# mynameisfiber/baton

Hardware: NVIDIA H100
Metric: federated local samples/sec (whole box), ResNet-18 FedAvg, synthetic non-IID 32x32 shards (higher is better)
Workload: dtype bf16

## Files before the change

### baton_b200/build_ext.py

```python
from __future__ import annotations

import os
import shutil
import subprocess
import sys
import sysconfig
import time
from concurrent.futures import ThreadPoolExecutor

HERE = os.path.dirname(os.path.abspath(__file__))
CSRC = os.path.join(HERE, "csrc")
BUILD = os.path.join(HERE, "csrc", "build")
TRACE = os.environ.get("BATON_BUILD_TRACE") == "1"
if TRACE:
    BUILD = os.path.join(HERE, "csrc", "build_trace")
TARGET = os.path.join(HERE, "_C_trace.so" if TRACE else "_C.so")

CU_SOURCES = ["gemm_wgmma.cu", "gemm_fp8.cu", "quant.cu", "attention.cu", "im2col_tma.cu", "gemm_simt.cu", "fedavg.cu", "elementwise.cu", "conv.cu", "norm.cu", "loss.cu"]
HEADERS = ["ptx.cuh", "launch.h", "pdl.cuh", "mx.cuh", "sgd.cuh", "dp.cuh"]
NVCC_FLAGS = ["-gencode", "arch=compute_90a,code=sm_90a", "-lineinfo", "-O3", "-std=c++17",
              "-Xcompiler", "-fPIC", "--use_fast_math", "-Xptxas", "-v"]
if os.environ.get("BATON_BUILD_PHASE_TIMING") == "1":
    NVCC_FLAGS.append("-DB200_FEDAVG_PHASE_TIMING")
if TRACE:
    NVCC_FLAGS += ["-DB200_TRACE", "-DB200_FEDAVG_PHASE_TIMING"]


def _nvcc() -> str:
    for cand in (os.environ.get("CUDA_HOME", "") + "/bin/nvcc", "/usr/local/cuda/bin/nvcc", shutil.which("nvcc") or ""):
        if cand and os.path.exists(cand):
            return cand
    raise RuntimeError("nvcc not found")


# ... 72 lines not shown
```

### baton_b200/csrc/bindings.cpp

```cpp
#include <ATen/cuda/CUDAContext.h>
#include <c10/cuda/CUDAGuard.h>
#include <torch/extension.h>

#include <optional>
#include <vector>

#include "launch.h"

namespace {

inline cudaStream_t cur_stream() { return at::cuda::getCurrentCUDAStream().stream(); }
inline void check(int rc, const char* what) {
  TORCH_CHECK(rc == 0, "baton_b200::", what, " failed with code ", rc,
              rc > 0 ? std::string(" (") + cudaGetErrorString(static_cast<cudaError_t>(rc)) + ")" : std::string());
}
inline const void* cptr(const at::Tensor& t) { return t.data_ptr(); }
inline void* ptr(at::Tensor& t) { return t.data_ptr(); }
template <class T>
inline T* opt_ptr(const std::optional<at::Tensor>& t) {
  return (t.has_value() && t->defined()) ? reinterpret_cast<T*>(t->data_ptr()) : nullptr;
}
#define CHECK_CUDA(x) TORCH_CHECK((x).is_cuda(), #x " must be a CUDA tensor")

inline const float* prox_anchor(const std::optional<at::Tensor>& anchor, int64_t numel, const at::Tensor& hyper) {
// ... 31 lines not shown
              "affine epilogue: fp32 [N] scale / shift");
  long long ldr = 0;
  if (residual.has_value() && residual->defined()) {
    CHECK_CUDA(*residual);
    TORCH_CHECK(residual->scalar_type() == at::kBFloat16 && residual->stride(-1) == 1 && residual->size(-1) == N &&
                    residual->numel() >= rows * N,
                "affine epilogue: bf16 [rows, N] residual with unit inner stride");
    ldr = residual->dim() >= 2 ? residual->stride(-2) : N;
  }
  return B200AffineEpilogue{scale->data_ptr<float>(), shift->data_ptr<float>(), opt_ptr<const void>(residual), ldr,
                            relu ? 1 : 0};
}

extern "C" {
#define B200_TRACE_TUS(X) X(gemm_wgmma) X(gemm_fp8) X(quant) X(attention) X(im2col_tma) X(gemm_simt) X(fedavg) \
  X(elementwise) X(conv) X(norm) X(loss)
#define B200_DECL(tu) int b200_trace_set_##tu(unsigned long long* p);
B200_TRACE_TUS(B200_DECL)
#undef B200_DECL
}
bool trace_set(const std::optional<at::Tensor>& buf) {
  unsigned long long* p = nullptr;
  if (buf.has_value() && buf->defined()) {
    CHECK_CUDA(*buf);
    TORCH_CHECK(buf->scalar_type() == at::kLong && buf->is_contiguous() && buf->numel() >= 4, "trace buffer: int64 [2+2n]");
    p = reinterpret_cast<unsigned long long*>(buf->data_ptr());
  }
  int rc = 0;
#define B200_SET(tu) rc |= b200_trace_set_##tu(p);
  B200_TRACE_TUS(B200_SET)
#undef B200_SET
// ... 116 lines not shown
  return true;
}
bool conv_igemm_dgrad(const at::Tensor& dy, const at::Tensor& w, at::Tensor dx, int64_t kh, int64_t kw, int64_t pad,
                      int64_t cluster_k, int64_t force_bn) {
  CHECK_CUDA(dy); CHECK_CUDA(w); CHECK_CUDA(dx);
  TORCH_CHECK(dy.scalar_type() == at::kBFloat16 && w.scalar_type() == at::kBFloat16 && dx.scalar_type() == at::kBFloat16 &&
              dy.dim() == 4 && dx.dim() == 4 && dy.is_contiguous() && w.is_contiguous() && dx.is_contiguous());
  const c10::cuda::CUDAGuard guard(dy.device());
  const int rc = b200_conv_igemm_dgrad(cptr(dy), cptr(w), ptr(dx), static_cast<int>(dx.size(0)), static_cast<int>(dx.size(1)),
                                       static_cast<int>(dx.size(2)), static_cast<int>(dx.size(3)), static_cast<int>(dy.size(3)),
                                       static_cast<int>(kh), static_cast<int>(kw), static_cast<int>(pad),
                                       static_cast<int>(dy.size(1)), static_cast<int>(dy.size(2)),
                                       static_cast<int>(cluster_k), static_cast<int>(force_bn), cur_stream());
  if (rc == -2) return false;
  check(rc, "conv_igemm_dgrad");
  return true;
}
bool conv_igemm_dgrad_s2(const at::Tensor& dy, const at::Tensor& w, at::Tensor dx, int64_t kh, int64_t kw,
                         const std::vector<int64_t>& ntaps, const std::vector<int64_t>& taps, int64_t force_bn) {
  CHECK_CUDA(dy); CHECK_CUDA(w); CHECK_CUDA(dx);
  TORCH_CHECK(dy.scalar_type() == at::kBFloat16 && w.scalar_type() == at::kBFloat16 && dx.scalar_type() == at::kBFloat16 &&
              dy.dim() == 4 && dx.dim() == 4 && dy.is_contiguous() && w.is_contiguous() && dx.is_contiguous());
  TORCH_CHECK(ntaps.size() == 4 && taps.size() == 16, "conv_igemm_dgrad_s2: 4 classes x 4 taps");
  int nt[4], tw[16];
  for (int i = 0; i < 4; ++i) nt[i] = static_cast<int>(ntaps[i]);
  for (int i = 0; i < 16; ++i) tw[i] = static_cast<int>(taps[i]);
  const c10::cuda::CUDAGuard guard(dy.device());
  const int rc = b200_conv_igemm_dgrad_s2(cptr(dy), cptr(w), ptr(dx), static_cast<int>(dx.size(0)),
                                          static_cast<int>(dx.size(1)), static_cast<int>(dx.size(2)),
                                          static_cast<int>(dx.size(3)), static_cast<int>(dy.size(3)), static_cast<int>(kh),
// ... 534 lines not shown
}

PYBIND11_MODULE(TORCH_EXTENSION_NAME, m) {
  m.doc() = "baton_b200 sm_90a kernels";
  m.attr("MAX_RANKS") = B200_MAX_RANKS;
  m.def("gemm", &gemm);
  m.def("trace_set", &trace_set);
  m.def("attention_fwd", &attention_fwd);
  m.def("attention_bwd", &attention_bwd);
  m.def("bn_bwd_cluster", &bn_bwd_cluster);
  m.def("im2col_tma_probe", &im2col_tma_probe);
  m.def("conv_igemm_fwd", &conv_igemm_fwd);
  m.def("conv_igemm_wgrad", &conv_igemm_wgrad);
  m.def("conv_igemm_dgrad", &conv_igemm_dgrad);
  m.def("conv_igemm_dgrad_s2", &conv_igemm_dgrad_s2);
  m.def("gemm_batched", &gemm_batched);
  m.def("gemm_fp8", &gemm_fp8);
  m.def("quant_mx_rows", &quant_mx_rows);
  m.def("quant_mx_cols", &quant_mx_cols);
  m.def("dequant_mx", &dequant_mx);
  m.def("fused_sgd", &fused_sgd);
  m.def("fused_sgd_segments", &fused_sgd_segments);
  m.def("weighted_sum", &weighted_sum);
  m.def("fold_client", &fold_client);
  m.def("cast", &cast);
  m.def("gather_rows", &gather_rows);
  m.def("colsum", &colsum);
  m.def("add_bf16", &add_bf16);
  m.def("relu_bwd", &relu_bwd);
  m.def("gelu", &gelu);
// ... 31 lines not shown
```

### baton_b200/csrc/gemm_wgmma.cu

```cuda
#define B200_TU_TAG 1
#include "ptx.cuh"
#include "launch.h"
#include "pdl.cuh"
#include "sgd.cuh"

namespace b200 {

constexpr int BM = 128;
constexpr int BK = 64;
constexpr int WG_K = 16;
constexpr int GEMM_THREADS = 384;
constexpr int CONSUMER_WARPS = 8;
constexpr int CONSUMER_THREADS = 32 * CONSUMER_WARPS;
constexpr int MAX_STAGES = 8;
constexpr int S2_MAX_TAPS = 4;

struct GemmParams {
  int M, N, K;
  void* D;
  long long ldd;
  const float* bias;
  int out_fp32;
  int act;
  float* col_stats;
// ... 51 lines not shown
  static constexpr int STAGE_BYTES = A_BYTES + B_BYTES;
  static constexpr int PART_PITCH = BN + 4;
  static constexpr int PART_BYTES = BM * PART_PITCH * 4;
};

__device__ __forceinline__ float apply_act(float v, int act) {
  if (act == 1) return fmaxf(v, 0.f);
  if (act == 2) {
    const float k0 = 0.7978845608028654f, k1 = 0.044715f;
    float t = tanhf(k0 * (v + k1 * v * v * v));
    return 0.5f * v * (1.f + t);
  }
  return v;
}

__device__ __forceinline__ uint32_t cluster_ctarank() {
  uint32_t r;
  asm volatile("mov.u32 %0, %%cluster_ctarank;" : "=r"(r));
  return r;
}
__device__ __forceinline__ void cluster_sync_all() {
  asm volatile("barrier.cluster.arrive.release.aligned;" ::: "memory");
  asm volatile("barrier.cluster.wait.acquire.aligned;" ::: "memory");
}
__device__ __forceinline__ float4 ld_dsmem_f4(uint32_t local_smem_addr, uint32_t cta_rank) {
  uint32_t remote;
  asm volatile("mapa.shared::cluster.u32 %0, %1, %2;" : "=r"(remote) : "r"(local_smem_addr), "r"(cta_rank));
  float4 v;
  asm volatile("ld.shared::cluster.v4.f32 {%0, %1, %2, %3}, [%4];"
               : "=f"(v.x), "=f"(v.y), "=f"(v.z), "=f"(v.w)
               : "r"(remote)
               : "memory");
  return v;
}

#define COLSUM_STEP(OFF, HALF)                                                  \
  {                                                                             \
    const bool upper = (lane & (OFF)) != 0;                                     \
    _Pragma("unroll") for (int i = 0; i < (HALF); ++i) {                        \
      const float keep = upper ? t[i + (HALF)] : t[i];                          \
      const float send = upper ? t[i] : t[i + (HALF)];                          \
      t[i] = keep + __shfl_xor_sync(0xffffffffu, send, (OFF));                  \
    }                                                                           \
  }
__device__ __forceinline__ float warp_colsum32(float (&t)[32]) {
  const uint32_t lane = lane_id();
  COLSUM_STEP(16, 16) COLSUM_STEP(8, 8) COLSUM_STEP(4, 4) COLSUM_STEP(2, 2) COLSUM_STEP(1, 1)
  return t[0];
}
#undef COLSUM_STEP
__device__ __forceinline__ void accumulate_col_stats(const GemmParams& p, int col0, const float (&v)[32]) {
  float s[32], q[32];
#pragma unroll
  for (int j = 0; j < 32; ++j) {
    const float r = __bfloat162float(__float2bfloat16_rn(v[j]));
    s[j] = r;
    q[j] = r * r;
  }
  const float cs = warp_colsum32(s), cq = warp_colsum32(q);
  const int col = col0 + static_cast<int>(lane_id());
  if (col < p.N) {
    atomicAdd(p.col_stats + col, cs);
    atomicAdd(p.col_stats + p.N + col, cq);
  }
}

__device__ __forceinline__ void stage_col_stats(float* sbuf, int BNv, int c, const float (&v)[32]) {
  float s[32], q[32];
#pragma unroll
  for (int j = 0; j < 32; ++j) {
    const float r = __bfloat162float(__float2bfloat16_rn(v[j]));
    s[j] = r;
    q[j] = r * r;
  }
  const float cs = warp_colsum32(s), cq = warp_colsum32(q);
  const int lane = static_cast<int>(lane_id());
  sbuf[c + lane] = cs;
  sbuf[BNv + c + lane] = cq;
}

template <int NV, int ACT, bool BIAS>
__device__ __forceinline__ void transform_chunk_t(const GemmParams& p, int col0, float (&v)[NV]) {
  float b[NV];
  if (BIAS) {
    if (col0 + NV <= p.N && ((reinterpret_cast<uintptr_t>(p.bias + col0) & 15) == 0)) {
#pragma unroll
      for (int j = 0; j < NV; j += 4) {
        const float4 t = __ldg(reinterpret_cast<const float4*>(p.bias + col0 + j));
        b[j] = t.x; b[j + 1] = t.y; b[j + 2] = t.z; b[j + 3] = t.w;
      }
    } else {
#pragma unroll
      for (int j = 0; j < NV; ++j) b[j] = (col0 + j) < p.N ? __ldg(p.bias + col0 + j) : 0.f;
// ... 964 lines not shown
  if (le != cudaSuccess) return static_cast<int>(le);
  return static_cast<int>(cudaGetLastError());
}

}

extern "C" int b200_encode_map2_bf16(void* map, const void* base, long long rows, long long cols, long long ld,
                                     int box_cols, int box_rows) {
  return b200::make_map(reinterpret_cast<CUtensorMap*>(map), base, rows, cols, ld, box_cols, box_rows);
}
extern "C" int b200_encode_map4_bf16(void* map, const void* base, long long rows, long long cols, long long ld,
                                     long long inner, long long s_inner, long long outer, long long s_outer,
                                     int box_cols, int box_rows) {
  return b200::make_map4(reinterpret_cast<CUtensorMap*>(map), base, rows, cols, ld, inner, s_inner, outer, s_outer,
                         box_cols, box_rows);
}

extern "C" int b200_gemm_bf16(const void* a, const void* b, void* d, const float* bias, int M, int N, int K,
                              long long lda, long long ldb, long long ldd, int a_mn, int b_mn, int out_fp32, int act,
                              int split_k, int accumulate, float alpha, const uint32_t* tile_flags,
                              uint32_t flag_epoch, long long flag_elem_off, int flag_tile_elems,
                              long long flag_bias_off, int force_bn, float* col_stats, const uint32_t* flag_epoch_ptr,
                              const B200SgdEpilogue* sgd, const B200AffineEpilogue* affine, cudaStream_t stream) {
  using namespace b200;
  if (M <= 0 || N <= 0 || K <= 0) return 0;
  if (sgd != nullptr && (!accumulate || !out_fp32 || !a_mn || !b_mn || bias != nullptr || act != 0 || alpha != 1.0f ||
                         col_stats != nullptr || tile_flags != nullptr))
    return B200_SGD_EPILOGUE_DECLINED;
  if (affine != nullptr && (sgd != nullptr || accumulate || out_fp32 || bias != nullptr || act != 0 || alpha != 1.0f ||
                            col_stats != nullptr || tile_flags != nullptr || split_k > 1 || !affine_ok(*affine, N)))
// ... 311 lines not shown
```

### baton_b200/csrc/launch.h

```cpp
#pragma once
#include <cuda_runtime.h>
#include <stdint.h>

#define B200_MAX_RANKS 16

extern "C" {

struct B200SgdEpilogue {
  float* theta;
  void* theta_bf16;
  float* mom;
  const float* hyper;
  int nesterov;
  const float* anchor;
};
#define B200_SGD_EPILOGUE_DECLINED (-6)

struct B200AffineEpilogue {
  const float* scale;
  const float* shift;
  const void* residual;
  long long ldr;
  int relu;
};
// ... 10 lines not shown
                           long long d_outer, long long d_inner, int accumulate, cudaStream_t stream);
int b200_attention_fwd(const void* qkv, void* out, void* probs, int B, int S, int H, int dh, float scale,
                       cudaStream_t stream);
int b200_attention_bwd(const void* qkv, const void* dout, const void* probs, void* dqkv, int B, int S, int H, int dh,
                       float scale, cudaStream_t stream);
int b200_conv_igemm_fwd(const void* x, const void* w, void* y, int N, int H, int W, int Cin, int Cout, int KH, int KW,
                        int stride, int pad, int Ho, int Wo, int cluster_k, int force_bn, float* col_stats,
                        const B200AffineEpilogue* affine, cudaStream_t stream);
int b200_conv_igemm_dgrad(const void* dy, const void* w, void* dx, int N, int H, int W, int Cin, int Cout, int KH, int KW,
                          int pad, int Ho, int Wo, int cluster_k, int force_bn, cudaStream_t stream);
int b200_conv_igemm_dgrad_s2(const void* dy, const void* w, void* dx, int N, int H, int W, int Cin, int Cout, int KH,
                             int KW, int Ho, int Wo, const int* ntaps, const int* taps, int force_bn, cudaStream_t stream);
int b200_conv_igemm_wgrad(const void* dy, const void* x, float* dw, int N, int H, int W, int Cin, int Cout, int KH, int KW,
                          int stride, int pad, int Ho, int Wo, int split_k, int force_bn, const B200SgdEpilogue* sgd,
                          cudaStream_t stream);
int b200_im2col_tma_probe(const void* x, void* col, int N, int H, int W, int C, int KH, int KW, int stride, int pad,
                          int Ho, int Wo, cudaStream_t stream);
int b200_gemm_fp8(const void* a, const void* b, void* d, const float* bias, const void* sfa, const void* sfb, int M, int N,
                  int K, long long lda, long long ldb, long long ldd, int out_fp32, int act, int split_k, int accumulate,
                  float alpha, cudaStream_t stream);
int b200_quant_mx_rows(const void* x, void* q, void* sf, long long R, int C, long long ld_in, int Cp, cudaStream_t stream);
int b200_quant_mx_cols(const void* x, void* q, void* sf, long long R, int C, long long ld_in, long long Rp,
                       cudaStream_t stream);
int b200_dequant_mx(const void* q, const void* sf, float* out, long long R, int C, int Cp, cudaStream_t stream);
int b200_gemm_simt(const void* a, const void* b, void* d, const float* bias, int M, int N, int K, long long lda,
                   long long ldb, long long ldd, int a_mn, int b_mn, int out_fp32, int act, int accumulate,
                   float alpha, cudaStream_t stream);

int b200_fused_sgd(float* w, float* g, float* mom, void* w_bf16, long long n, const float* hyper, int zero_grad,
                   int nesterov, const unsigned long long* wire_slot, const float* pack_global,
// ... 126 lines not shown
```

### baton_b200/csrc/ptx.cuh

```cuda
#pragma once
#include <cuda.h>
#include <cuda_bf16.h>
#include <cuda_runtime.h>
#include <stdint.h>

namespace b200 {

__device__ __forceinline__ uint32_t smem_u32(const void* p) {
  return static_cast<uint32_t>(__cvta_generic_to_shared(p));
}
__device__ __forceinline__ uint32_t lane_id() {
  uint32_t l;
  asm volatile("mov.u32 %0, %%laneid;" : "=r"(l));
  return l;
}
__device__ __forceinline__ bool elect_one() {
  uint32_t pred;
  asm volatile(
      "{\n\t.reg .pred p;\n\t"
      "elect.sync _|p, 0xffffffff;\n\t"
      "selp.u32 %0, 1, 0, p;\n\t}"
      : "=r"(pred));
  return pred != 0;
}
// ... 37 lines not shown
__device__ __forceinline__ void tma_load_2d(void* smem_dst, const CUtensorMap* m, uint64_t* bar, int c0,
                                            int c1) {
  asm volatile(
      "cp.async.bulk.tensor.2d.shared::cluster.global.mbarrier::complete_tx::bytes [%0], [%1, {%3, %4}], [%2];"
      ::"r"(smem_u32(smem_dst)),
      "l"(reinterpret_cast<uint64_t>(m)), "r"(smem_u32(bar)), "r"(c0), "r"(c1)
      : "memory");
}

__device__ __forceinline__ void tma_load_4d(void* smem_dst, const CUtensorMap* m, uint64_t* bar, int c0, int c1,
                                            int c2, int c3) {
  asm volatile(
      "cp.async.bulk.tensor.4d.shared::cluster.global.mbarrier::complete_tx::bytes [%0], [%1, {%3, %4, %5, %6}], [%2];"
      ::"r"(smem_u32(smem_dst)),
      "l"(reinterpret_cast<uint64_t>(m)), "r"(smem_u32(bar)), "r"(c0), "r"(c1), "r"(c2), "r"(c3)
      : "memory");
}

__device__ __forceinline__ void tma_load_im2col_4d(void* smem_dst, const CUtensorMap* m, uint64_t* bar, int c, int w, int h,
                                                   int n, int off_w, int off_h) {
  asm volatile(
      "cp.async.bulk.tensor.4d.shared::cluster.global.im2col.mbarrier::complete_tx::bytes"
      " [%0], [%1, {%3, %4, %5, %6}], [%2], {%7, %8};" ::"r"(smem_u32(smem_dst)),
      "l"(reinterpret_cast<uint64_t>(m)), "r"(smem_u32(bar)), "r"(c), "r"(w), "r"(h), "r"(n),
      "h"(static_cast<uint16_t>(off_w)), "h"(static_cast<uint16_t>(off_h))
      : "memory");
}
__device__ __forceinline__ void wgmma_fence() { asm volatile("wgmma.fence.sync.aligned;" ::: "memory"); }
__device__ __forceinline__ void wgmma_commit() { asm volatile("wgmma.commit_group.sync.aligned;" ::: "memory"); }
template <int N>
// ... 38 lines not shown
      "{"
      "%0, %1, %2, %3, %4, %5, %6, %7, %8, %9, %10, %11, %12, %13, %14, %15, "
      "%16, %17, %18, %19, %20, %21, %22, %23, %24, %25, %26, %27, %28, %29, %30, %31, "
      "%32, %33, %34, %35, %36, %37, %38, %39, %40, %41, %42, %43, %44, %45, %46, %47, "
      "%48, %49, %50, %51, %52, %53, %54, %55, %56, %57, %58, %59, %60, %61, %62, %63"
      "}, %64, %65, p, 1, 1, %67, %68;\n\t}"
      : "+f"(d[0]), "+f"(d[1]), "+f"(d[2]), "+f"(d[3]), "+f"(d[4]), "+f"(d[5]), "+f"(d[6]), "+f"(d[7]),
        "+f"(d[8]), "+f"(d[9]), "+f"(d[10]), "+f"(d[11]), "+f"(d[12]), "+f"(d[13]), "+f"(d[14]), "+f"(d[15]),
        "+f"(d[16]), "+f"(d[17]), "+f"(d[18]), "+f"(d[19]), "+f"(d[20]), "+f"(d[21]), "+f"(d[22]), "+f"(d[23]),
        "+f"(d[24]), "+f"(d[25]), "+f"(d[26]), "+f"(d[27]), "+f"(d[28]), "+f"(d[29]), "+f"(d[30]), "+f"(d[31]),
        "+f"(d[32]), "+f"(d[33]), "+f"(d[34]), "+f"(d[35]), "+f"(d[36]), "+f"(d[37]), "+f"(d[38]), "+f"(d[39]),
        "+f"(d[40]), "+f"(d[41]), "+f"(d[42]), "+f"(d[43]), "+f"(d[44]), "+f"(d[45]), "+f"(d[46]), "+f"(d[47]),
        "+f"(d[48]), "+f"(d[49]), "+f"(d[50]), "+f"(d[51]), "+f"(d[52]), "+f"(d[53]), "+f"(d[54]), "+f"(d[55]),
        "+f"(d[56]), "+f"(d[57]), "+f"(d[58]), "+f"(d[59]), "+f"(d[60]), "+f"(d[61]), "+f"(d[62]), "+f"(d[63])
      : "l"(da), "l"(db), "r"(scale_d), "n"(TA), "n"(TB));
}
__device__ __forceinline__ void wgmma_e4m3_n64(float (&d)[32], uint64_t da, uint64_t db, uint32_t scale_d) {
  asm volatile(
      "{\n\t.reg .pred p;\n\tsetp.ne.b32 p, %34, 0;\n\t"
      "wgmma.mma_async.sync.aligned.m64n64k32.f32.e4m3.e4m3 "
      "{"
      "%0, %1, %2, %3, %4, %5, %6, %7, %8, %9, %10, %11, %12, %13, %14, %15, "
      "%16, %17, %18, %19, %20, %21, %22, %23, %24, %25, %26, %27, %28, %29, %30, %31"
      "}, %32, %33, p, 1, 1;\n\t}"
      : "+f"(d[0]), "+f"(d[1]), "+f"(d[2]), "+f"(d[3]), "+f"(d[4]), "+f"(d[5]), "+f"(d[6]), "+f"(d[7]),
        "+f"(d[8]), "+f"(d[9]), "+f"(d[10]), "+f"(d[11]), "+f"(d[12]), "+f"(d[13]), "+f"(d[14]), "+f"(d[15]),
        "+f"(d[16]), "+f"(d[17]), "+f"(d[18]), "+f"(d[19]), "+f"(d[20]), "+f"(d[21]), "+f"(d[22]), "+f"(d[23]),
        "+f"(d[24]), "+f"(d[25]), "+f"(d[26]), "+f"(d[27]), "+f"(d[28]), "+f"(d[29]), "+f"(d[30]), "+f"(d[31])
      : "l"(da), "l"(db), "r"(scale_d));
}
// ... 133 lines not shown
```

### baton_b200/ops/functional.py

```python
from __future__ import annotations

from typing import List, Optional, Sequence, Tuple

import torch

from ._ext import load

BF16 = torch.bfloat16
NUM_SMS = 132


def _pitch(t: torch.Tensor) -> int:
    assert t.dim() == 2 and (t.stride(1) == 1 or t.shape[1] == 1), "GEMM operand must have unit inner stride"
    return t.stride(0) if t.shape[0] > 1 else max(t.stride(0), t.shape[1])


def _tma_ok(t: torch.Tensor) -> bool:
    return t.dtype == BF16 and _pitch(t) % 8 == 0 and t.data_ptr() % 16 == 0


def pick_bn(M: int, N: int) -> int:
    m_tiles = (M + 127) // 128
    if N >= 128 and m_tiles * ((N + 127) // 128) >= NUM_SMS:
        return 128
# ... 237 lines not shown


def round_up(x: int, m: int) -> int:
    return (x + m - 1) // m * m


def im2col(x: torch.Tensor, kh: int, kw: int, stride: int, pad: int) -> Tuple[torch.Tensor, int, int, int]:
    n, h, w, c = x.shape
    ho, wo = conv_out_size(h, kh, stride, pad), conv_out_size(w, kw, stride, pad)
    kp = round_up(kh * kw * c, 8)
    col = torch.empty((n * ho * wo, kp), dtype=BF16, device=x.device)
    load().im2col(x, col, n, h, w, c, kh, kw, stride, pad, ho, wo, kp)
    return col, ho, wo, kp


def conv_igemm_fwd(x: torch.Tensor, w2d: torch.Tensor, kh: int, kw: int, stride: int, pad: int,
                   col_stats: Optional[torch.Tensor] = None, affine: Optional[dict] = None,
                   cluster_k: Optional[int] = None, force_bn: int = 0,
                   out: Optional[torch.Tensor] = None) -> Optional[torch.Tensor]:
    n, h, w, c = x.shape
    cout = w2d.shape[0]
    if c % 64 or w2d.shape[1] != kh * kw * c or not x.is_contiguous() or not w2d.is_contiguous():
        return None
    ho, wo = conv_out_size(h, kh, stride, pad), conv_out_size(w, kw, stride, pad)
    M, K = n * ho * wo, kh * kw * c
    bn = force_bn or pick_bn(M, cout)
    if cluster_k is None:
        cluster_k = pick_cluster_k(M, cout, K, bn)
    y = out if out is not None else torch.empty((M, cout), dtype=BF16, device=x.device)
    af = affine or {}
    ok = load().conv_igemm_fwd(x, w2d, y, kh, kw, stride, pad, ho, wo, cluster_k, bn, col_stats, af.get("scale"),
                               af.get("shift"), af.get("residual"), bool(af.get("relu", False)))
    return y if ok else None


S2_MAX_TAPS = 4


def conv_s2_dgrad_taps(kh: int, kw: int, pad: int, ho: int, wo: int) -> Optional[List[List[Tuple[int, int, int]]]]:
    classes = []
# ... 7 lines not shown
                for s in range(kw):
                    if (b + pad - s) % 2:
                        continue
                    dq = (b + pad - s) // 2
                    if dp < 0 or dq < 0:
                        return None
                    if dp < ho and dq < wo:
                        taps.append((r * kw + s, dp, dq))
            if len(taps) > S2_MAX_TAPS:
                return None
            classes.append(taps)
    return classes


def conv_igemm_dgrad(dy: torch.Tensor, w2d: torch.Tensor, in_shape, kh: int, kw: int, pad: int, stride: int = 1,
                     out: Optional[torch.Tensor] = None) -> Optional[torch.Tensor]:
    n, h, w, c = in_shape
    cout = dy.shape[-1]
    if c % 64 or cout % 64 or w2d.shape[1] != kh * kw * c or not dy.is_contiguous() or not w2d.is_contiguous():
        return None
    if stride == 1:
        M, K = n * h * w, kh * kw * cout
        bn = pick_bn(M, c)
        dx = out if out is not None else torch.empty((n, h, w, c), dtype=BF16, device=dy.device)
        ok = load().conv_igemm_dgrad(dy, w2d, dx, kh, kw, pad, pick_cluster_k(M, c, K, bn), bn)
        return dx if ok else None
    if stride != 2:
        return None
    ho, wo = dy.shape[1], dy.shape[2]
    classes = conv_s2_dgrad_taps(kh, kw, pad, ho, wo)
    if classes is None:
        return None
    bn = pick_bn(4 * n * ho * wo, c)
    words = [[t | dp << 16 | dq << 24 for t, dp, dq in taps] + [0] * (S2_MAX_TAPS - len(taps)) for taps in classes]
    dx = out if out is not None else torch.empty((n, h, w, c), dtype=BF16, device=dy.device)
# ... 182 lines not shown
```

### baton_b200/utils/trace.py

```python
from __future__ import annotations

import collections
import os
import re
from typing import Dict, List, Tuple

import torch

_TUS = ["?", "gemm_wgmma", "gemm_fp8", "quant", "attention", "im2col_tma", "gemm_simt", "fedavg", "elementwise",
        "conv", "norm", "loss"]
_CSRC = os.path.join(os.path.dirname(os.path.dirname(os.path.abspath(__file__))), "csrc")
_NAME_CACHE: Dict[int, str] = {}


POINT_BASE = 5_000_000_000


def point_label(tag: int) -> str:
    tu, line = divmod(int(tag) - POINT_BASE, 100000)
    try:
        with open(os.path.join(_CSRC, _TUS[tu] + ".cu")) as f:
            src = f.readlines()
        text = src[line - 1]
        return text.split("//", 1)[1].strip() if "//" in text else "{}:{}".format(_TUS[tu], line)
    except (OSError, IndexError):
# ... 14 lines not shown
                m = re.search(r"(\w+)\s*\(", " ".join(s.strip() for s in src[i:i + 4]).split("__global__", 1)[1]
                              .replace("__launch_bounds__", " ").replace("__cluster_dims__", " "))
                cands = re.findall(r"([A-Za-z_]\w*)\s*\(", " ".join(s.strip() for s in src[i:i + 4]))
                cands = [c for c in cands if c not in ("__launch_bounds__", "__cluster_dims__")]
                if cands:
                    name = cands[0]
                elif m:
                    name = m.group(1)
                break
    except OSError:
        pass
    _NAME_CACHE[tag] = name
    return name


class KernelTrace:
    def __init__(self, capacity: int = 1 << 16, device=None):
        from ..ops._ext import load
        self.C = load()
        self.device = torch.device(device or "cuda:0")
        self.capacity = capacity
        self.buf = torch.zeros(2 + 2 * capacity, dtype=torch.int64, device=self.device)
        self.buf[1] = capacity
        self.enabled = False

    def start(self) -> bool:
        self.buf[0] = 0
        self.enabled = bool(self.C.trace_set(self.buf))
        return self.enabled

    def stop(self) -> None:
        torch.cuda.synchronize(self.device)
        self.C.trace_set(None)

    def records(self) -> List[Tuple[int, int]]:
        torch.cuda.synchronize(self.device)
        host = self.buf.cpu()
        n = min(int(host[0]), self.capacity)
        rec = host[2: 2 + 2 * n].view(n, 2).tolist()
        rec.sort()
        return [(int(t), int(tag)) for t, tag in rec]

    def timeline(self) -> List[dict]:
        rec = [r for r in self.records() if abs(r[1]) < POINT_BASE]
        resident = collections.defaultdict(list)
        rows = []
        for t, tag in rec:
            if tag < 0:
                resident[-tag].append(t)
            else:
                pre = resident[tag].pop(0) if resident[tag] else t
                rows.append({"t_ns": t, "tag": tag, "name": kernel_name(tag), "early_ns": t - pre})
        for a, b in zip(rows, rows[1:]):
            a["slot_ns"] = b["t_ns"] - a["t_ns"]
        if rows:
            rows[-1]["slot_ns"] = 0
        return rows

    def points(self) -> List[Tuple[int, str]]:
        out = []
        for t, tag in self.records():
            if tag >= POINT_BASE:
                out.append((t, "    . " + point_label(tag)))
            elif tag > 0:
                out.append((t, "> " + kernel_name(tag)))
            else:
                out.append((t, "  (resident) " + kernel_name(tag)))
        return out

    def summary(self, skip_first: int = 0) -> List[str]:
        rows = self.timeline()[skip_first:]
        tot = collections.defaultdict(float)
# ... 13 lines not shown
```

Baseline: 198,900.

## Add halo-tile implicit-GEMM kernel for small 3x3 stride-1 64-channel convs

Adds a conv_halo kernel for 3x3, stride-1, pad-1, 64-channel convolutions on small spatial maps, such as ResNet-18 layer1 at small resolutions. Each block loads a padded halo of whole images into shared memory once via a 4D TMA box and feeds the nine taps to register-sourced wgmma through ldmatrix. This replaces the im2col-expanded operand traffic of the existing path. Weight tiles can be multicast across a 2- or 4-CTA cluster, and the kernel is used by default in forward and dgrad whenever eligible. In exchange, each kernel launch encodes its tensor maps on the host, and the kernel holds one block per SM with a large shared-memory footprint.

```diff
diff --git a/baton_b200/build_ext.py b/baton_b200/build_ext.py
--- a/baton_b200/build_ext.py
+++ b/baton_b200/build_ext.py
@@ -16,8 +16,8 @@
     BUILD = os.path.join(HERE, "csrc", "build_trace")
 TARGET = os.path.join(HERE, "_C_trace.so" if TRACE else "_C.so")
 
-CU_SOURCES = ["gemm_wgmma.cu", "gemm_fp8.cu", "quant.cu", "attention.cu", "im2col_tma.cu", "gemm_simt.cu", "fedavg.cu", "elementwise.cu", "conv.cu", "norm.cu", "loss.cu"]
-HEADERS = ["ptx.cuh", "launch.h", "pdl.cuh", "mx.cuh", "sgd.cuh", "dp.cuh"]
+CU_SOURCES = ["gemm_wgmma.cu", "gemm_fp8.cu", "quant.cu", "attention.cu", "im2col_tma.cu", "gemm_simt.cu", "fedavg.cu", "elementwise.cu", "conv.cu", "norm.cu", "loss.cu", "conv_halo.cu"]
+HEADERS = ["ptx.cuh", "launch.h", "pdl.cuh", "mx.cuh", "sgd.cuh", "dp.cuh", "epilogue.cuh"]
 NVCC_FLAGS = ["-gencode", "arch=compute_90a,code=sm_90a", "-lineinfo", "-O3", "-std=c++17",
               "-Xcompiler", "-fPIC", "--use_fast_math", "-Xptxas", "-v"]
 if os.environ.get("BATON_BUILD_PHASE_TIMING") == "1":
diff --git a/baton_b200/csrc/bindings.cpp b/baton_b200/csrc/bindings.cpp
--- a/baton_b200/csrc/bindings.cpp
+++ b/baton_b200/csrc/bindings.cpp
@@ -69,7 +69,7 @@
 
 extern "C" {
 #define B200_TRACE_TUS(X) X(gemm_wgmma) X(gemm_fp8) X(quant) X(attention) X(im2col_tma) X(gemm_simt) X(fedavg) \
-  X(elementwise) X(conv) X(norm) X(loss)
+  X(elementwise) X(conv) X(norm) X(loss) X(conv_halo)
 #define B200_DECL(tu) int b200_trace_set_##tu(unsigned long long* p);
 B200_TRACE_TUS(B200_DECL)
 #undef B200_DECL
@@ -216,6 +216,26 @@
                                        static_cast<int>(cluster_k), static_cast<int>(force_bn), cur_stream());
   if (rc == -2) return false;
   check(rc, "conv_igemm_dgrad");
+  return true;
+}
+bool conv_halo(const at::Tensor& src, const at::Tensor& w, at::Tensor out, bool dgrad, int64_t mc,
+               const std::optional<at::Tensor>& col_stats) {
+  CHECK_CUDA(src); CHECK_CUDA(w); CHECK_CUDA(out);
+  TORCH_CHECK(src.scalar_type() == at::kBFloat16 && w.scalar_type() == at::kBFloat16 && out.scalar_type() == at::kBFloat16 &&
+              src.dim() == 4 && src.size(3) == 64 && src.is_contiguous() && w.is_contiguous() && out.is_contiguous());
+  const int64_t rows = src.size(0) * src.size(1) * src.size(2);
+  TORCH_CHECK(rows > 0 && out.numel() % rows == 0, "conv_halo: out must hold [N*H*W, Nout] elements");
+  const int64_t nout = out.numel() / rows;
+  TORCH_CHECK(w.numel() == (dgrad ? 64 * 9 * nout : nout * 9 * 64), "conv_halo: w must be [Cout, 9*Cin]");
+  TORCH_CHECK(dgrad ? !col_stats.has_value()
+                    : (!col_stats.has_value() || (col_stats->scalar_type() == at::kFloat && col_stats->numel() >= 2 * nout)),
+              "conv_halo: col_stats is a [2 Cout] fp32 buffer of the forward");
+  const c10::cuda::CUDAGuard guard(src.device());
+  const int rc = b200_conv_halo(cptr(src), cptr(w), ptr(out), static_cast<int>(src.size(0)), static_cast<int>(src.size(1)),
+                                static_cast<int>(src.size(2)), static_cast<int>(nout), dgrad ? 1 : 0,
+                                static_cast<int>(mc), opt_ptr<float>(col_stats), cur_stream());
+  if (rc == -2) return false;
+  check(rc, "conv_halo");
   return true;
 }
 bool conv_igemm_dgrad_s2(const at::Tensor& dy, const at::Tensor& w, at::Tensor dx, int64_t kh, int64_t kw,
@@ -780,6 +800,7 @@
   m.def("conv_igemm_wgrad", &conv_igemm_wgrad);
   m.def("conv_igemm_dgrad", &conv_igemm_dgrad);
   m.def("conv_igemm_dgrad_s2", &conv_igemm_dgrad_s2);
+  m.def("conv_halo", &conv_halo);
   m.def("gemm_batched", &gemm_batched);
   m.def("gemm_fp8", &gemm_fp8);
   m.def("quant_mx_rows", &quant_mx_rows);
diff --git a/baton_b200/csrc/conv_halo.cu b/baton_b200/csrc/conv_halo.cu
--- /dev/null
+++ b/baton_b200/csrc/conv_halo.cu
@@ -0,0 +1,246 @@
+#define B200_TU_TAG 12
+#include "ptx.cuh"
+#include "epilogue.cuh"
+#include "launch.h"
+#include "pdl.cuh"
+
+namespace b200 {
+
+constexpr int HALO_BM = 64;
+constexpr int HALO_BN = 64;
+constexpr int HALO_TAPS = 9;
+constexpr int HALO_THREADS = 256;
+constexpr int HALO_CONSUMERS = 128;
+constexpr int HALO_SLOT_BYTES = 64 * 64 * 2;
+constexpr int HALO_PART_PITCH = HALO_BN + 4;
+constexpr int HALO_MAX_SMEM = 227 * 1024;
+
+struct HaloParams {
+  int M, N;
+  int H, W;
+  __nv_bfloat16* D;
+  float* col_stats;
+  int ncol;
+  int mc;
+  int halo_bytes;
+};
+
+__host__ __device__ constexpr int halo_fixed_bytes() {
+  return HALO_TAPS * HALO_SLOT_BYTES + 16 * 8 + 4 * HALO_BN * 4 + 1024;
+}
+
+template <bool DGRAD>
+__global__ void __launch_bounds__(HALO_THREADS, 1)
+conv_halo_kernel(const __grid_constant__ CUtensorMap tmX, const __grid_constant__ CUtensorMap tmW, const HaloParams p) {
+  extern __shared__ __align__(1024) uint8_t smem_raw[];
+  uint8_t* smem = reinterpret_cast<uint8_t*>((reinterpret_cast<uintptr_t>(smem_raw) + 1023) & ~uintptr_t(1023));
+  uint8_t* halo = smem;
+  uint8_t* bslot = smem + p.halo_bytes;
+  uint64_t* bar = reinterpret_cast<uint64_t*>(bslot + HALO_TAPS * HALO_SLOT_BYTES);
+  float* cstat = reinterpret_cast<float*>(bar + 16);
+
+  griddep_launch_dependents();
+  const int warp = threadIdx.x >> 5;
+  const int m0 = blockIdx.y * HALO_BM;
+  const int n0 = blockIdx.x * HALO_BN;
+  const int hw = p.H * p.W;
+
+  if (warp == 0 && elect_one()) {
+    tma_prefetch_desc(&tmX);
+    tma_prefetch_desc(&tmW);
+    for (int i = 0; i < 1 + HALO_TAPS; ++i) mbar_init(&bar[i], 1);
+    fence_barrier_init();
+  }
+  __syncthreads();
+  if (p.mc > 1) cluster_sync_all();
+  griddep_wait();
+
+  if (warp == 0) {
+    if (elect_one()) {
+      const int imgs = HALO_BM / hw;
+      mbar_expect_tx(&bar[0], imgs * (p.H + 2) * (p.W + 2) * 128);
+      tma_load_4d(halo, &tmX, &bar[0], 0, -1, -1, m0 / hw);
+      const int rows = 64 / p.mc;
+      const int rank = p.mc > 1 ? static_cast<int>(cluster_ctarank()) : 0;
+      const uint16_t mask = static_cast<uint16_t>((1u << p.mc) - 1);
+#pragma unroll 1
+      for (int t = 0; t < HALO_TAPS; ++t) {
+        mbar_expect_tx(&bar[1 + t], HALO_SLOT_BYTES);
+        uint8_t* dst = bslot + t * HALO_SLOT_BYTES + rank * rows * 128;
+        const int c0 = DGRAD ? (HALO_TAPS - 1 - t) * p.ncol + n0 : t * 64;
+        const int c1 = DGRAD ? rank * rows : n0 + rank * rows;
+        if (p.mc > 1)
+          tma_load_2d_mc(dst, &tmW, &bar[1 + t], c0, c1, mask);
+        else
+          tma_load_2d(dst, &tmW, &bar[1 + t], c0, c1);
+      }
+    }
+  } else if (warp >= 4) {
+    const int ew = warp - 4;
+    const int lane = static_cast<int>(lane_id());
+    const int m = 16 * ew + (lane & 15);
+    const int img = m / hw, rem = m - img * hw;
+    const int oi = rem / p.W, oj = rem - oi * p.W;
+    const int hp = p.W + 2;
+    const int hrow0 = (img * (p.H + 2) + oi) * hp + oj;
+    const uint32_t halo_a = smem_u32(halo);
+    const int half = lane >> 4;
+    auto load_a = [&](uint32_t (&a)[4][4], int t) {
+      const int r = t / 3, s = t - 3 * r;
+      const int hrow = hrow0 + r * hp + s;
+      const uint32_t row_addr = halo_a + static_cast<uint32_t>(hrow) * 128u;
+#pragma unroll
+      for (int kk = 0; kk < 4; ++kk) ldmatrix_x4(a[kk], row_addr + ((((2 * kk + half) ^ hrow) & 7) << 4));
+    };
+
+    float acc[32];
+#pragma unroll
+    for (int j = 0; j < 32; ++j) acc[j] = 0.f;
+    uint32_t a[2][4][4];
+    mbar_wait(&bar[0], 0);
+    load_a(a[0], 0);
+#pragma unroll
+    for (int t = 0; t < HALO_TAPS; ++t) {
+      mbar_wait(&bar[1 + t], 0);
+      const uint32_t sb = smem_u32(bslot + t * HALO_SLOT_BYTES);
+      wgmma_fence();
+#pragma unroll
+      for (int kk = 0; kk < 4; ++kk) {
+        const uint64_t bd = DGRAD ? gmma_desc_sw128(sb + kk * 2048, 8192, 1024) : gmma_desc_sw128(sb + kk * 32, 16, 1024);
+        wgmma_bf16_n64_rs<DGRAD ? 1 : 0>(acc, a[t & 1][kk], bd, 1u);
+      }
+      wgmma_commit();
+      if (t + 1 < HALO_TAPS) {
+        wgmma_wait<1>();
+        load_a(a[(t + 1) & 1], t + 1);
+      }
+    }
+    wgmma_wait<0>();
+    wgmma_fence_operands(acc);
+    if (threadIdx.x == 128) TRACE_POINT();
+
+    named_bar_sync(1, HALO_CONSUMERS);
+    float* part = reinterpret_cast<float*>(smem);
+    wg_store_acc<HALO_BN>(acc, part, HALO_PART_PITCH, 0);
+    named_bar_sync(1, HALO_CONSUMERS);
+    const int q = ew & 1;
+    const int c = (ew >> 1) * 32;
+    const int lrow = q * 32 + lane;
+    const int row = m0 + lrow;
+    const int col0 = n0 + c;
+    float* sstat = cstat + q * 2 * HALO_BN;
+    const bool want_stats = p.col_stats != nullptr;
+    if (col0 >= p.N) {
+      if (want_stats) { sstat[c + lane] = 0.f; sstat[HALO_BN + c + lane] = 0.f; }
+    } else {
+      uint32_t r[32];
+      acc_ld_row32(part + lrow * HALO_PART_PITCH + c, r);
+      float v[32];
+#pragma unroll
+      for (int j = 0; j < 32; ++j) v[j] = __uint_as_float(r[j]);
+      if (want_stats) stage_col_stats(sstat, HALO_BN, c, v);
+      if (row < p.M) {
+        __nv_bfloat16* d = p.D + static_cast<size_t>(row) * p.N + col0;
+        if (col0 + 32 <= p.N && (p.N % 8) == 0) {
+#pragma unroll
+          for (int j = 0; j < 32; j += 8) {
+            uint4 o;
+            o.x = pack_bf16x2(v[j], v[j + 1]);
+            o.y = pack_bf16x2(v[j + 2], v[j + 3]);
+            o.z = pack_bf16x2(v[j + 4], v[j + 5]);
+            o.w = pack_bf16x2(v[j + 6], v[j + 7]);
+            *reinterpret_cast<uint4*>(d + j) = o;
+          }
+        } else {
+          _Pragma("unroll") for (int j = 0; j < 32; ++j) if (col0 + j < p.N) d[j] = __float2bfloat16_rn(v[j]);
+        }
+      }
+    }
+    if (want_stats) {
+      named_bar_sync(1, HALO_CONSUMERS);
+      for (int i = threadIdx.x - 128; i < 2 * HALO_BN; i += HALO_CONSUMERS) {
+        const int col = i < HALO_BN ? i : i - HALO_BN;
+        if (n0 + col < p.N)
+          atomicAdd(p.col_stats + (i < HALO_BN ? 0 : p.N) + n0 + col,
+                    cstat[i] + cstat[2 * HALO_BN + i]);
+      }
+    }
+  }
+}
+
+template <bool DGRAD>
+static int launch_halo(const CUtensorMap& tx, const CUtensorMap& tw, const HaloParams& p, dim3 grid, int smem,
+                cudaStream_t stream) {
+  static bool configured = false;
+  if (!configured) {
+    cudaError_t e = cudaFuncSetAttribute(conv_halo_kernel<DGRAD>, cudaFuncAttributeMaxDynamicSharedMemorySize,
+                                         HALO_MAX_SMEM);
+    if (e != cudaSuccess) return static_cast<int>(e);
+    configured = true;
+  }
+  cudaLaunchConfig_t cfg = {};
+  cfg.gridDim = grid;
+  cfg.blockDim = dim3(HALO_THREADS);
+  cfg.dynamicSmemBytes = smem;
+  cfg.stream = stream;
+  cudaLaunchAttribute attr[2];
+  int na = 0;
+  if (pdl_enabled()) {
+    attr[na].id = cudaLaunchAttributeProgrammaticStreamSerialization;
+    attr[na].val.programmaticStreamSerializationAllowed = 1;
+    ++na;
+  }
+  if (p.mc > 1) {
+    attr[na].id = cudaLaunchAttributeClusterDimension;
+    attr[na].val.clusterDim.x = 1;
+    attr[na].val.clusterDim.y = p.mc;
+    attr[na].val.clusterDim.z = 1;
+    ++na;
+  }
+  cfg.attrs = attr;
+  cfg.numAttrs = na;
+  cudaError_t le = cudaLaunchKernelEx(&cfg, conv_halo_kernel<DGRAD>, tx, tw, p);
+  if (le != cudaSuccess) return static_cast<int>(le);
+  return static_cast<int>(cudaGetLastError());
+}
+
+}
+
+extern "C" int b200_encode_map2_bf16(void* map, const void* base, long long rows, long long cols, long long ld,
+                                     int box_cols, int box_rows);
+extern "C" int b200_encode_map4_box_bf16(void* map, const void* base, const long long* dims,
+                                         const long long* stride_bytes, const int* box);
+
+extern "C" int b200_conv_halo(const void* src, const void* w, void* out, int N, int H, int W, int Nout, int dgrad, int mc,
+                              float* col_stats, cudaStream_t stream) {
+  using namespace b200;
+  const long long M = static_cast<long long>(N) * H * W;
+  if (M <= 0 || Nout <= 0) return 0;
+  const int hw = H * W;
+  const long long m_tiles = (M + HALO_BM - 1) / HALO_BM;
+  if (hw <= 0 || HALO_BM % hw != 0 || H + 2 > 256 || W + 2 > 256 || M > (1ll << 30) || Nout % 8 != 0 ||
+      (dgrad && Nout % 64 != 0) || (mc != 1 && mc != 2 && mc != 4) || m_tiles % mc != 0 ||
+      (reinterpret_cast<uintptr_t>(src) & 15) || (reinterpret_cast<uintptr_t>(w) & 15) ||
+      (reinterpret_cast<uintptr_t>(out) & 15))
+    return -2;
+  const int imgs = HALO_BM / hw;
+  const int halo_bytes = (imgs * (H + 2) * (W + 2) * 128 + 1023) / 1024 * 1024;
+  const int smem = halo_bytes + halo_fixed_bytes();
+  if (smem > HALO_MAX_SMEM) return -2;
+  CUtensorMap tx, tw;
+  const long long dims[4] = {64, W, H, N};
+  const long long strides[3] = {64 * 2, static_cast<long long>(W) * 64 * 2, static_cast<long long>(hw) * 64 * 2};
+  const int box[4] = {64, W + 2, H + 2, imgs};
+  int rc = b200_encode_map4_box_bf16(&tx, src, dims, strides, box);
+  if (rc) return rc;
+  const long long wrows = dgrad ? 64 : Nout, wcols = dgrad ? 9ll * Nout : 9ll * 64;
+  rc = b200_encode_map2_bf16(&tw, w, wrows, wcols, wcols, 64, 64 / mc);
+  if (rc) return rc;
+  HaloParams p;
+  p.M = static_cast<int>(M); p.N = Nout; p.H = H; p.W = W; p.D = reinterpret_cast<__nv_bfloat16*>(out);
+  p.col_stats = col_stats; p.ncol = Nout; p.mc = mc; p.halo_bytes = halo_bytes;
+  dim3 grid((Nout + HALO_BN - 1) / HALO_BN, static_cast<unsigned>(m_tiles), 1);
+  return dgrad ? launch_halo<true>(tx, tw, p, grid, smem, stream) : launch_halo<false>(tx, tw, p, grid, smem, stream);
+}
+
+B200_TRACE_REGISTER(conv_halo)
diff --git a/baton_b200/csrc/epilogue.cuh b/baton_b200/csrc/epilogue.cuh
--- /dev/null
+++ b/baton_b200/csrc/epilogue.cuh
@@ -0,0 +1,46 @@
+#pragma once
+#include "ptx.cuh"
+
+namespace b200 {
+
+__device__ __forceinline__ uint32_t cluster_ctarank() {
+  uint32_t r;
+  asm volatile("mov.u32 %0, %%cluster_ctarank;" : "=r"(r));
+  return r;
+}
+__device__ __forceinline__ void cluster_sync_all() {
+  asm volatile("barrier.cluster.arrive.release.aligned;" ::: "memory");
+  asm volatile("barrier.cluster.wait.acquire.aligned;" ::: "memory");
+}
+
+#define COLSUM_STEP(OFF, HALF)                                                  \
+  {                                                                             \
+    const bool upper = (lane & (OFF)) != 0;                                     \
+    _Pragma("unroll") for (int i = 0; i < (HALF); ++i) {                        \
+      const float keep = upper ? t[i + (HALF)] : t[i];                          \
+      const float send = upper ? t[i] : t[i + (HALF)];                          \
+      t[i] = keep + __shfl_xor_sync(0xffffffffu, send, (OFF));                  \
+    }                                                                           \
+  }
+__device__ __forceinline__ float warp_colsum32(float (&t)[32]) {
+  const uint32_t lane = lane_id();
+  COLSUM_STEP(16, 16) COLSUM_STEP(8, 8) COLSUM_STEP(4, 4) COLSUM_STEP(2, 2) COLSUM_STEP(1, 1)
+  return t[0];
+}
+#undef COLSUM_STEP
+
+__device__ __forceinline__ void stage_col_stats(float* sbuf, int BNv, int c, const float (&v)[32]) {
+  float s[32], q[32];
+#pragma unroll
+  for (int j = 0; j < 32; ++j) {
+    const float r = __bfloat162float(__float2bfloat16_rn(v[j]));
+    s[j] = r;
+    q[j] = r * r;
+  }
+  const float cs = warp_colsum32(s), cq = warp_colsum32(q);
+  const int lane = static_cast<int>(lane_id());
+  sbuf[c + lane] = cs;
+  sbuf[BNv + c + lane] = cq;
+}
+
+}
diff --git a/baton_b200/csrc/gemm_wgmma.cu b/baton_b200/csrc/gemm_wgmma.cu
--- a/baton_b200/csrc/gemm_wgmma.cu
+++ b/baton_b200/csrc/gemm_wgmma.cu
@@ -1,5 +1,6 @@
 #define B200_TU_TAG 1
 #include "ptx.cuh"
+#include "epilogue.cuh"
 #include "launch.h"
 #include "pdl.cuh"
 #include "sgd.cuh"
@@ -89,15 +90,6 @@
   return v;
 }
 
-__device__ __forceinline__ uint32_t cluster_ctarank() {
-  uint32_t r;
-  asm volatile("mov.u32 %0, %%cluster_ctarank;" : "=r"(r));
-  return r;
-}
-__device__ __forceinline__ void cluster_sync_all() {
-  asm volatile("barrier.cluster.arrive.release.aligned;" ::: "memory");
-  asm volatile("barrier.cluster.wait.acquire.aligned;" ::: "memory");
-}
 __device__ __forceinline__ float4 ld_dsmem_f4(uint32_t local_smem_addr, uint32_t cta_rank) {
   uint32_t remote;
   asm volatile("mapa.shared::cluster.u32 %0, %1, %2;" : "=r"(remote) : "r"(local_smem_addr), "r"(cta_rank));
@@ -109,21 +101,6 @@
   return v;
 }
 
-#define COLSUM_STEP(OFF, HALF)                                                  \
-  {                                                                             \
-    const bool upper = (lane & (OFF)) != 0;                                     \
-    _Pragma("unroll") for (int i = 0; i < (HALF); ++i) {                        \
-      const float keep = upper ? t[i + (HALF)] : t[i];                          \
-      const float send = upper ? t[i] : t[i + (HALF)];                          \
-      t[i] = keep + __shfl_xor_sync(0xffffffffu, send, (OFF));                  \
-    }                                                                           \
-  }
-__device__ __forceinline__ float warp_colsum32(float (&t)[32]) {
-  const uint32_t lane = lane_id();
-  COLSUM_STEP(16, 16) COLSUM_STEP(8, 8) COLSUM_STEP(4, 4) COLSUM_STEP(2, 2) COLSUM_STEP(1, 1)
-  return t[0];
-}
-#undef COLSUM_STEP
 __device__ __forceinline__ void accumulate_col_stats(const GemmParams& p, int col0, const float (&v)[32]) {
   float s[32], q[32];
 #pragma unroll
@@ -138,20 +115,6 @@
     atomicAdd(p.col_stats + col, cs);
     atomicAdd(p.col_stats + p.N + col, cq);
   }
-}
-
-__device__ __forceinline__ void stage_col_stats(float* sbuf, int BNv, int c, const float (&v)[32]) {
-  float s[32], q[32];
-#pragma unroll
-  for (int j = 0; j < 32; ++j) {
-    const float r = __bfloat162float(__float2bfloat16_rn(v[j]));
-    s[j] = r;
-    q[j] = r * r;
-  }
-  const float cs = warp_colsum32(s), cq = warp_colsum32(q);
-  const int lane = static_cast<int>(lane_id());
-  sbuf[c + lane] = cs;
-  sbuf[BNv + c + lane] = cq;
 }
 
 template <int NV, int ACT, bool BIAS>
@@ -1146,6 +1109,22 @@
                                      int box_cols, int box_rows) {
   return b200::make_map4(reinterpret_cast<CUtensorMap*>(map), base, rows, cols, ld, inner, s_inner, outer, s_outer,
                          box_cols, box_rows);
+}
+extern "C" int b200_encode_map4_box_bf16(void* map, const void* base, const long long* dims, const long long* stride_bytes,
+                                         const int* box) {
+  b200::EncodeTiledFn fn = b200::get_encode_fn();
+  if (fn == nullptr) return -1;
+  cuuint64_t gdim[4], gstr[3];
+  cuuint32_t bx[4], estr[4] = {1, 1, 1, 1};
+  for (int i = 0; i < 4; ++i) {
+    gdim[i] = static_cast<cuuint64_t>(dims[i]);
+    bx[i] = static_cast<cuuint32_t>(box[i]);
+    if (i < 3) gstr[i] = static_cast<cuuint64_t>(stride_bytes[i]);
+  }
+  CUresult r = fn(reinterpret_cast<CUtensorMap*>(map), CU_TENSOR_MAP_DATA_TYPE_BFLOAT16, 4, const_cast<void*>(base), gdim,
+                  gstr, bx, estr, CU_TENSOR_MAP_INTERLEAVE_NONE, CU_TENSOR_MAP_SWIZZLE_128B,
+                  CU_TENSOR_MAP_L2_PROMOTION_L2_256B, CU_TENSOR_MAP_FLOAT_OOB_FILL_NONE);
+  return r == CUDA_SUCCESS ? 0 : static_cast<int>(r);
 }
 
 extern "C" int b200_gemm_bf16(const void* a, const void* b, void* d, const float* bias, int M, int N, int K,
diff --git a/baton_b200/csrc/launch.h b/baton_b200/csrc/launch.h
--- a/baton_b200/csrc/launch.h
+++ b/baton_b200/csrc/launch.h
@@ -48,6 +48,8 @@
 int b200_conv_igemm_wgrad(const void* dy, const void* x, float* dw, int N, int H, int W, int Cin, int Cout, int KH, int KW,
                           int stride, int pad, int Ho, int Wo, int split_k, int force_bn, const B200SgdEpilogue* sgd,
                           cudaStream_t stream);
+int b200_conv_halo(const void* src, const void* w, void* out, int N, int H, int W, int Nout, int dgrad, int mc,
+                   float* col_stats, cudaStream_t stream);
 int b200_im2col_tma_probe(const void* x, void* col, int N, int H, int W, int C, int KH, int KW, int stride, int pad,
                           int Ho, int Wo, cudaStream_t stream);
 int b200_gemm_fp8(const void* a, const void* b, void* d, const float* bias, const void* sfa, const void* sfb, int M, int N,
diff --git a/baton_b200/csrc/ptx.cuh b/baton_b200/csrc/ptx.cuh
--- a/baton_b200/csrc/ptx.cuh
+++ b/baton_b200/csrc/ptx.cuh
@@ -75,6 +75,15 @@
       "cp.async.bulk.tensor.4d.shared::cluster.global.mbarrier::complete_tx::bytes [%0], [%1, {%3, %4, %5, %6}], [%2];"
       ::"r"(smem_u32(smem_dst)),
       "l"(reinterpret_cast<uint64_t>(m)), "r"(smem_u32(bar)), "r"(c0), "r"(c1), "r"(c2), "r"(c3)
+      : "memory");
+}
+
+__device__ __forceinline__ void tma_load_2d_mc(void* smem_dst, const CUtensorMap* m, uint64_t* bar, int c0, int c1,
+                                               uint16_t cta_mask) {
+  asm volatile(
+      "cp.async.bulk.tensor.2d.shared::cluster.global.mbarrier::complete_tx::bytes.multicast::cluster"
+      " [%0], [%1, {%3, %4}], [%2], %5;" ::"r"(smem_u32(smem_dst)),
+      "l"(reinterpret_cast<uint64_t>(m)), "r"(smem_u32(bar)), "r"(c0), "r"(c1), "h"(cta_mask)
       : "memory");
 }
 
@@ -143,6 +152,27 @@
         "+f"(d[48]), "+f"(d[49]), "+f"(d[50]), "+f"(d[51]), "+f"(d[52]), "+f"(d[53]), "+f"(d[54]), "+f"(d[55]),
         "+f"(d[56]), "+f"(d[57]), "+f"(d[58]), "+f"(d[59]), "+f"(d[60]), "+f"(d[61]), "+f"(d[62]), "+f"(d[63])
       : "l"(da), "l"(db), "r"(scale_d), "n"(TA), "n"(TB));
+}
+template <int TB>
+__device__ __forceinline__ void wgmma_bf16_n64_rs(float (&d)[32], const uint32_t (&a)[4], uint64_t db, uint32_t scale_d) {
+  asm volatile(
+      "{\n\t.reg .pred p;\n\tsetp.ne.b32 p, %37, 0;\n\t"
+      "wgmma.mma_async.sync.aligned.m64n64k16.f32.bf16.bf16 "
+      "{"
+      "%0, %1, %2, %3, %4, %5, %6, %7, %8, %9, %10, %11, %12, %13, %14, %15, "
+      "%16, %17, %18, %19, %20, %21, %22, %23, %24, %25, %26, %27, %28, %29, %30, %31"
+      "}, {%32, %33, %34, %35}, %36, p, 1, 1, %38;\n\t}"
+      : "+f"(d[0]), "+f"(d[1]), "+f"(d[2]), "+f"(d[3]), "+f"(d[4]), "+f"(d[5]), "+f"(d[6]), "+f"(d[7]),
+        "+f"(d[8]), "+f"(d[9]), "+f"(d[10]), "+f"(d[11]), "+f"(d[12]), "+f"(d[13]), "+f"(d[14]), "+f"(d[15]),
+        "+f"(d[16]), "+f"(d[17]), "+f"(d[18]), "+f"(d[19]), "+f"(d[20]), "+f"(d[21]), "+f"(d[22]), "+f"(d[23]),
+        "+f"(d[24]), "+f"(d[25]), "+f"(d[26]), "+f"(d[27]), "+f"(d[28]), "+f"(d[29]), "+f"(d[30]), "+f"(d[31])
+      : "r"(a[0]), "r"(a[1]), "r"(a[2]), "r"(a[3]), "l"(db), "r"(scale_d), "n"(TB));
+}
+__device__ __forceinline__ void ldmatrix_x4(uint32_t (&r)[4], uint32_t smem_addr) {
+  asm volatile("ldmatrix.sync.aligned.m8n8.x4.shared.b16 {%0, %1, %2, %3}, [%4];"
+               : "=r"(r[0]), "=r"(r[1]), "=r"(r[2]), "=r"(r[3])
+               : "r"(smem_addr)
+               : "memory");
 }
 __device__ __forceinline__ void wgmma_e4m3_n64(float (&d)[32], uint64_t da, uint64_t db, uint32_t scale_d) {
   asm volatile(
diff --git a/baton_b200/ops/functional.py b/baton_b200/ops/functional.py
--- a/baton_b200/ops/functional.py
+++ b/baton_b200/ops/functional.py
@@ -275,16 +275,51 @@
     return col, ho, wo, kp
 
 
+HALO_BM = 64
+_HALO_MAX_SMEM = 227 * 1024
+
+
+def halo_smem_bytes(h: int, w: int) -> int:
+    halo = round_up((HALO_BM // (h * w)) * (h + 2) * (w + 2) * 128, 1024)
+    return halo + 9 * 8192 + 16 * 8 + 4 * 64 * 4 + 1024
+
+
+def halo_eligible(kh: int, kw: int, stride: int, pad: int, c: int, h: int, w: int, affine: Optional[dict] = None) -> bool:
+    return (kh == 3 and kw == 3 and stride == 1 and pad == 1 and c == 64 and h * w <= HALO_BM and
+            HALO_BM % (h * w) == 0 and affine is None and halo_smem_bytes(h, w) <= _HALO_MAX_SMEM)
+
+
+def halo_cluster(m_rows: int) -> int:
+    tiles = (m_rows + HALO_BM - 1) // HALO_BM
+    return 4 if tiles % 4 == 0 else 2 if tiles % 2 == 0 else 1
+
+
+def _conv_path(path: Optional[str], eligible: bool) -> str:
+    if path is None:
+        return "halo" if eligible else "im2col"
+    if path not in ("halo", "im2col"):
+        raise ValueError("path must be None, 'halo' or 'im2col', not {!r}".format(path))
+    if path == "halo" and not eligible:
+        raise ValueError("the halo kernel does not take this convolution (see halo_eligible)")
+    return path
+
+
 def conv_igemm_fwd(x: torch.Tensor, w2d: torch.Tensor, kh: int, kw: int, stride: int, pad: int,
                    col_stats: Optional[torch.Tensor] = None, affine: Optional[dict] = None,
                    cluster_k: Optional[int] = None, force_bn: int = 0,
-                   out: Optional[torch.Tensor] = None) -> Optional[torch.Tensor]:
+                   out: Optional[torch.Tensor] = None, path: Optional[str] = None,
+                   mc: Optional[int] = None) -> Optional[torch.Tensor]:
     n, h, w, c = x.shape
     cout = w2d.shape[0]
     if c % 64 or w2d.shape[1] != kh * kw * c or not x.is_contiguous() or not w2d.is_contiguous():
         return None
     ho, wo = conv_out_size(h, kh, stride, pad), conv_out_size(w, kw, stride, pad)
     M, K = n * ho * wo, kh * kw * c
+    if _conv_path(path, halo_eligible(kh, kw, stride, pad, c, h, w, affine) and cout % 8 == 0) == "halo":
+        y = out if out is not None else torch.empty((M, cout), dtype=BF16, device=x.device)
+        if not load().conv_halo(x, w2d, y, False, mc or halo_cluster(M), col_stats):
+            raise RuntimeError("conv_halo declined a convolution halo_eligible admits")
+        return y
     bn = force_bn or pick_bn(M, cout)
     if cluster_k is None:
         cluster_k = pick_cluster_k(M, cout, K, bn)
@@ -322,11 +357,17 @@
 
 
 def conv_igemm_dgrad(dy: torch.Tensor, w2d: torch.Tensor, in_shape, kh: int, kw: int, pad: int, stride: int = 1,
-                     out: Optional[torch.Tensor] = None) -> Optional[torch.Tensor]:
+                     out: Optional[torch.Tensor] = None, path: Optional[str] = None,
+                     mc: Optional[int] = None) -> Optional[torch.Tensor]:
     n, h, w, c = in_shape
     cout = dy.shape[-1]
     if c % 64 or cout % 64 or w2d.shape[1] != kh * kw * c or not dy.is_contiguous() or not w2d.is_contiguous():
         return None
+    if _conv_path(path, halo_eligible(kh, kw, stride, pad, cout, h, w)) == "halo":
+        dx = out if out is not None else torch.empty((n, h, w, c), dtype=BF16, device=dy.device)
+        if not load().conv_halo(dy, w2d, dx, True, mc or halo_cluster(n * h * w), None):
+            raise RuntimeError("conv_halo declined a convolution halo_eligible admits")
+        return dx
     if stride == 1:
         M, K = n * h * w, kh * kw * cout
         bn = pick_bn(M, c)
diff --git a/baton_b200/utils/trace.py b/baton_b200/utils/trace.py
--- a/baton_b200/utils/trace.py
+++ b/baton_b200/utils/trace.py
@@ -3,12 +3,12 @@
 import collections
 import os
 import re
-from typing import Dict, List, Tuple
+from typing import Callable, Dict, List, Tuple
 
 import torch
 
 _TUS = ["?", "gemm_wgmma", "gemm_fp8", "quant", "attention", "im2col_tma", "gemm_simt", "fedavg", "elementwise",
-        "conv", "norm", "loss"]
+        "conv", "norm", "loss", "conv_halo"]
 _CSRC = os.path.join(os.path.dirname(os.path.dirname(os.path.abspath(__file__))), "csrc")
 _NAME_CACHE: Dict[int, str] = {}
 
@@ -53,6 +53,25 @@
     return name
 
 
+def timeline_rows(records: List[Tuple[int, int]], name: Callable[[int], str] = kernel_name) -> List[dict]:
+    resident = collections.defaultdict(collections.deque)
+    rows = []
+    for t, tag in records:
+        if abs(tag) >= POINT_BASE:
+            continue
+        k = name(tag)
+        if tag < 0:
+            resident[k].append(t)
+        else:
+            pre = resident[k].popleft() if resident[k] else t
+            rows.append({"t_ns": t, "tag": tag, "name": k, "early_ns": t - pre})
+    for a, b in zip(rows, rows[1:]):
+        a["slot_ns"] = b["t_ns"] - a["t_ns"]
+    if rows:
+        rows[-1]["slot_ns"] = 0
+    return rows
+
+
 class KernelTrace:
     def __init__(self, capacity: int = 1 << 16, device=None):
         from ..ops._ext import load
@@ -81,20 +100,7 @@
         return [(int(t), int(tag)) for t, tag in rec]
 
     def timeline(self) -> List[dict]:
-        rec = [r for r in self.records() if abs(r[1]) < POINT_BASE]
-        resident = collections.defaultdict(list)
-        rows = []
-        for t, tag in rec:
-            if tag < 0:
-                resident[-tag].append(t)
-            else:
-                pre = resident[tag].pop(0) if resident[tag] else t
-                rows.append({"t_ns": t, "tag": tag, "name": kernel_name(tag), "early_ns": t - pre})
-        for a, b in zip(rows, rows[1:]):
-            a["slot_ns"] = b["t_ns"] - a["t_ns"]
-        if rows:
-            rows[-1]["slot_ns"] = 0
-        return rows
+        return timeline_rows(self.records())
 
     def points(self) -> List[Tuple[int, str]]:
         out = []
```

Result: faster. 205,600 (median of 6 runs) (+3.4%).
